# jinggqu/NextGen-UIA

Measured on AMD Instinct MI355X. Metric: images/sec fwd+bwd BiomedCLIP+Mona bs=256, higher is better.
Workload: dtype bf16

## Files before the change

### nextgen-uia_amd/csrc/wgrad.hip

```cpp
#include "uia_common.h"
#include "uia_kernels.h"

namespace {

typedef __attribute__((ext_vector_type(4))) short s16x4;
typedef __attribute__((ext_vector_type(8))) short s16x8;

__device__ __forceinline__ void glds16(const char* gsrc, char* lds_wave_base) {
    __builtin_amdgcn_global_load_lds((const __attribute__((address_space(1))) void*)gsrc,
                                     (__attribute__((address_space(3))) void*)lds_wave_base, 16, 0, 0);
}
__device__ __forceinline__ s16x4 lds_tr16(const char* p) {
    return __builtin_amdgcn_ds_read_tr16_b64_v4i16((__attribute__((address_space(3))) s16x4*)p);
}

constexpr int SLAB = 128;
#ifndef WG_CHUNK_SLABS
#define WG_CHUNK_SLABS 4
#endif
constexpr int CHUNK_SLABS = WG_CHUNK_SLABS;

#ifndef WG_MIN_WAVES
#define WG_MIN_WAVES 1
#endif
struct WgradGroups {
    const bf16_t* A[4];
    const bf16_t* B[4];
    float* dW[4];
    float* dbias[4];
    unsigned long long seed[4];
};

template <bool DROPB>
__global__ __launch_bounds__(256, DROPB ? 3 : WG_MIN_WAVES) void wgrad_bf16_kernel(int M, int I, int J, const WgradGroups gp, long lda, long ldb, float alpha,
                                                          long ldw, int i_valid, int j_valid, float drop_p, long drop_ld, int drop_col0) {
    extern __shared__ __attribute__((aligned(16))) char smem[];
    const bf16_t* __restrict__ A = gp.A[blockIdx.y];
    const bf16_t* __restrict__ B = gp.B[blockIdx.y];
    float* __restrict__ dW = gp.dW[blockIdx.y];
    float* __restrict__ dbias = gp.dbias[blockIdx.y];
    const unsigned long long drop_seed = gp.seed[blockIdx.y];
    char* As = smem;
    char* Bs = smem + SLAB * 128;
    const int tid = threadIdx.x, lane = tid & 63;
    const int wave = __builtin_amdgcn_readfirstlane(tid >> 6);
    const int tiles = (I / 64) * (J / 64);
    const int xcd = blockIdx.x & 7, slot = blockIdx.x >> 3;
    const int chunk = xcd + 8 * (slot / tiles), tile = slot % tiles;
    const int tj = tile % (J / 64), ti = tile / (J / 64);
    const int m_begin = chunk * (SLAB * CHUNK_SLABS);
    if (m_begin >= M) return;
    const int li = lane & 15, g = lane >> 4, qq = li >> 2, pp = li & 3;

    f32x4 acc[4][4];
#pragma unroll
    for (int a = 0; a < 4; ++a)
#pragma unroll
        for (int b = 0; b < 4; ++b) acc[a][b] = f32x4{0.f, 0.f, 0.f, 0.f};
    const bool want_bias = dbias != nullptr && tj == 0;
    f32x4 bacc[4] = {f32x4{0.f, 0.f, 0.f, 0.f}, f32x4{0.f, 0.f, 0.f, 0.f}, f32x4{0.f, 0.f, 0.f, 0.f}, f32x4{0.f, 0.f, 0.f, 0.f}};
    const bf16x8 ones = {(bf16_t)1.f, (bf16_t)1.f, (bf16_t)1.f, (bf16_t)1.f, (bf16_t)1.f, (bf16_t)1.f, (bf16_t)1.f, (bf16_t)1.f};

    const uint32_t drop_th = dropout_thresh16(drop_p);
    const float drop_inv = 1.0f / (1.0f - drop_p);
    const int trow = 32 * wave + 4 * g + qq;
    const int tsw = (trow >> 1) & 3;
    for (int sl = 0; sl < CHUNK_SLABS; ++sl) {
        const int m0 = m_begin + sl * SLAB;
        if (m0 >= M) break;
        __syncthreads();
        if constexpr (DROPB) {
            uint4 raw[SLAB / 32];
            uint32_t keep[SLAB / 32];
#pragma unroll
            for (int i = 0; i < SLAB / 32; ++i) {
                const int q = wave + 4 * i, r = 8 * q + (lane >> 3);
                int gm = m0 + r;
                gm = gm < M ? gm : M - 1;
                const int c = ((lane & 7) ^ (((r >> 1) & 3) << 1)) * 16;
                glds16((const char*)(A + (size_t)gm * lda + (size_t)ti * 64) + c, As + q * 1024);
                raw[i] = *(const uint4*)((const char*)(B + (size_t)gm * ldb + (size_t)tj * 64) + c);
            }
#pragma unroll
            for (int i = 0; i < SLAB / 32; ++i) {
                const int q = wave + 4 * i, r = 8 * q + (lane >> 3);
                int gm = m0 + r;
                gm = gm < M ? gm : M - 1;
                const int c = ((lane & 7) ^ (((r >> 1) & 3) << 1)) * 16;
                keep[i] = dropout_keep8(drop_seed, (uint32_t)(((size_t)gm * (size_t)drop_ld + (size_t)(drop_col0 + tj * 64 + (c >> 1))) >> 3), drop_th);
            }
#pragma unroll
            for (int i = 0; i < SLAB / 32; ++i) {
                const int q = wave + 4 * i;
                bf16x8 v = __builtin_bit_cast(bf16x8, raw[i]);
#pragma unroll
                for (int e = 0; e < 8; ++e) v[e] = (bf16_t)((keep[i] >> e) & 1u ? (float)v[e] * drop_inv : 0.f);
                *(bf16x8*)(Bs + q * 1024 + lane * 16) = v;
            }
        } else {
        for (int q = wave; q < SLAB / 8; q += 4) {
            const int r = 8 * q + (lane >> 3);
            int gm = m0 + r;
            gm = gm < M ? gm : M - 1;
            const int c = ((lane & 7) ^ (((r >> 1) & 3) << 1)) * 16;
            glds16((const char*)(A + (size_t)gm * lda + (size_t)ti * 64) + c, As + q * 1024);
            glds16((const char*)(B + (size_t)gm * ldb + (size_t)tj * 64) + c, Bs + q * 1024);
        }
        }
        asm volatile("s_waitcnt vmcnt(0)" ::: "memory");
        __syncthreads();
        const bool tail = m0 + SLAB > M;
        bf16x8 af[4], bfr[4];
#pragma unroll
        for (int t = 0; t < 4; ++t) {
            const int off = trow * 128 + ((t ^ tsw) << 5) + 8 * pp;
            s16x4 alo = lds_tr16(As + off), ahi = lds_tr16(As + off + 16 * 128);
            const s16x4 blo = lds_tr16(Bs + off), bhi = lds_tr16(Bs + off + 16 * 128);
            if (tail) {
#pragma unroll
                for (int e = 0; e < 4; ++e) {
                    if (m0 + 32 * wave + 4 * g + e >= M) alo[e] = 0;
                    if (m0 + 32 * wave + 16 + 4 * g + e >= M) ahi[e] = 0;
                }
            }
            const s16x8 av = {alo[0], alo[1], alo[2], alo[3], ahi[0], ahi[1], ahi[2], ahi[3]};
            const s16x8 bv = {blo[0], blo[1], blo[2], blo[3], bhi[0], bhi[1], bhi[2], bhi[3]};
            af[t] = __builtin_bit_cast(bf16x8, av);
            bfr[t] = __builtin_bit_cast(bf16x8, bv);
        }
#pragma unroll
        for (int a = 0; a < 4; ++a)
#pragma unroll
            for (int b = 0; b < 4; ++b) acc[a][b] = __builtin_amdgcn_mfma_f32_16x16x32_bf16(af[a], bfr[b], acc[a][b], 0, 0, 0);
        if (want_bias) {
#pragma unroll
            for (int a = 0; a < 4; ++a) bacc[a] = __builtin_amdgcn_mfma_f32_16x16x32_bf16(af[a], ones, bacc[a], 0, 0, 0);
        }
    }
    __syncthreads();
    float* red = (float*)smem;
    float* mine = red + (wave & 1) * 4096;
    if (wave < 2) {
#pragma unroll
        for (int a = 0; a < 4; ++a)
#pragma unroll
            for (int b = 0; b < 4; ++b)
#pragma unroll
                for (int r = 0; r < 4; ++r)
                    mine[(16 * a + 4 * g + r) * 64 + 16 * b + li] = acc[a][b][r];
    }
    __syncthreads();
    if (wave >= 2) {
#pragma unroll
        for (int a = 0; a < 4; ++a)
#pragma unroll
            for (int b = 0; b < 4; ++b)
#pragma unroll
                for (int r = 0; r < 4; ++r)
                    mine[(16 * a + 4 * g + r) * 64 + 16 * b + li] += acc[a][b][r];
    }
    __syncthreads();
#ifndef WG_NO_ATOMIC
    for (int e = tid; e < 4096; e += 256) {
        const float v = red[e] + red[4096 + e];
        const int i = ti * 64 + (e >> 6), j = tj * 64 + (e & 63);
        if (i < i_valid && j < j_valid) atomicAdd(dW + (size_t)i * ldw + j, v * alpha);
    }
#endif
    if (want_bias) {
        __syncthreads();
        if (li == 0) {
#pragma unroll
            for (int a = 0; a < 4; ++a)
#pragma unroll
                for (int r = 0; r < 4; ++r) red[wave * 64 + 16 * a + 4 * g + r] = bacc[a][r];
        }
        __syncthreads();
        if (tid < 64 && ti * 64 + tid < i_valid) atomicAdd(dbias + ti * 64 + tid, (red[tid] + red[64 + tid]) + (red[128 + tid] + red[192 + tid]));
    }
}

__global__ __launch_bounds__(256) void wgrad_f32_kernel(int M, int I, int J, const float* __restrict__ A, long lda,
                                                         const float* __restrict__ B, long ldb, float alpha,
                                                         float* __restrict__ dW, float* __restrict__ dbias, long ldw, int i_valid, int j_valid) {
    extern __shared__ __attribute__((aligned(16))) char smem[];
    const int tid = threadIdx.x, lane = tid & 63;
    const int wave = __builtin_amdgcn_readfirstlane(tid >> 6);
    const int tj = blockIdx.x % (J / 64), ti = blockIdx.x / (J / 64);
    const int m_begin = blockIdx.y * (SLAB * CHUNK_SLABS);
    const int m_end = min(M, m_begin + SLAB * CHUNK_SLABS);
    const int li = lane & 15, g = lane >> 4;
    f32x4 acc[4][4];
#pragma unroll
    for (int a = 0; a < 4; ++a)
#pragma unroll
        for (int b = 0; b < 4; ++b) acc[a][b] = f32x4{0.f, 0.f, 0.f, 0.f};
    float bsum = 0.f;
    for (int m = m_begin + 4 * wave; m < m_end; m += 16) {
        const int row = m + g;
        const bool ok = row < m_end;
        const int rr = ok ? row : m_end - 1;
        float av[4], bv[4];
#pragma unroll
        for (int t = 0; t < 4; ++t) {
            av[t] = ok ? A[(size_t)rr * lda + ti * 64 + 16 * t + li] : 0.f;
            bv[t] = B[(size_t)rr * ldb + tj * 64 + 16 * t + li];
            bsum += av[t];
        }
#pragma unroll
        for (int a = 0; a < 4; ++a)
#pragma unroll
            for (int b = 0; b < 4; ++b) acc[a][b] = __builtin_amdgcn_mfma_f32_16x16x4f32(av[a], bv[b], acc[a][b], 0, 0, 0);
        (void)bsum;
    }
    __syncthreads();
    float* red = (float*)smem;
#pragma unroll
    for (int a = 0; a < 4; ++a)
#pragma unroll
        for (int b = 0; b < 4; ++b)
#pragma unroll
            for (int r = 0; r < 4; ++r) red[wave * 4096 + (16 * a + 4 * g + r) * 64 + 16 * b + li] = acc[a][b][r];
    __syncthreads();
    for (int e = tid; e < 4096; e += 256) {
        const float v = red[e] + red[4096 + e] + red[8192 + e] + red[12288 + e];
        const int i = ti * 64 + (e >> 6), j = tj * 64 + (e & 63);
        if (i < i_valid && j < j_valid) atomicAdd(dW + (size_t)i * ldw + j, v * alpha);
    }
    if (dbias && tj == 0) {
        const int col = tid & 63, part = tid >> 6;
        float s = 0.f;
        for (int m = m_begin + part; m < m_end; m += 4) s += A[(size_t)m * lda + ti * 64 + col];
        __syncthreads();
        red[tid] = s;
        __syncthreads();
        if (tid < 64 && ti * 64 + tid < i_valid) atomicAdd(dbias + ti * 64 + tid, red[tid] + red[64 + tid] + red[128 + tid] + red[192 + tid]);
    }
}

}

int uia_wgrad_group_launch(hipStream_t stream, int dtype, int n, int M, int I, int J, const void* const* A, long lda, const void* const* B, long ldb, float alpha,
                            float* const* dW, float* const* dbias, long ldw, int i_valid, int j_valid, float drop_p, const uint64_t* drop_seed, long drop_ld, int drop_col0) {
    if (ldw == 0) { ldw = J; i_valid = I; j_valid = J; }
    UIA_CHECK_ARG(dtype == UIA_BF16 || dtype == UIA_F32, "uia_wgrad: bad dtype %d", dtype);
    UIA_CHECK_ARG(n >= 1 && n <= 4 && (n == 1 || dtype == UIA_BF16), "uia_wgrad_group: 1..4 problems per launch (bf16), got %d", n);
    UIA_CHECK_ARG(M > 0 && I > 0 && J > 0 && I % 64 == 0 && J % 64 == 0, "uia_wgrad: I=%d and J=%d must be multiples of 64 (M=%d)", I, J, M);
    const int esz = dtype == UIA_BF16 ? 2 : 4;
    UIA_CHECK_ARG((lda * esz) % 16 == 0 && (ldb * esz) % 16 == 0, "uia_wgrad: alignment");
    UIA_CHECK_ARG(lda >= I && ldb >= J, "uia_wgrad: leading dimension too small");
    UIA_CHECK_ARG(i_valid > 0 && i_valid <= I && j_valid > 0 && j_valid <= J && ldw >= j_valid, "uia_wgrad: valid extent %d x %d (ldw %ld) outside the padded %d x %d", i_valid, j_valid, ldw, I, J);
    WgradGroups gp = {};
    for (int g = 0; g < n; ++g) {
        UIA_CHECK_ARG(A[g] && B[g] && dW[g] && (uintptr_t)A[g] % 16 == 0 && (uintptr_t)B[g] % 16 == 0, "uia_wgrad: null or misaligned tensor (problem %d)", g);
        gp.A[g] = (const bf16_t*)A[g]; gp.B[g] = (const bf16_t*)B[g]; gp.dW[g] = dW[g]; gp.dbias[g] = dbias ? dbias[g] : nullptr; gp.seed[g] = drop_seed ? drop_seed[g] : 0;
    }
    const int chunks = (M + SLAB * CHUNK_SLABS - 1) / (SLAB * CHUNK_SLABS);
    const dim3 grid_f32((I / 64) * (J / 64), chunks);
    const dim3 grid(8 * ((chunks + 7) / 8) * (I / 64) * (J / 64), n);
    const int lds = 4 * 4096 * 4;
    const int lds_bf16 = 2 * SLAB * 128;
    static UiaDevOnce once_bf16, once_f32;
    UIA_CHECK_ARG(drop_p >= 0.f && drop_p < 1.f, "uia_wgrad: drop_p=%f outside [0, 1)", (double)drop_p);
    UIA_CHECK_ARG(drop_p == 0.f || (dtype == UIA_BF16 && drop_ld >= drop_col0 + J && drop_col0 >= 0 && drop_col0 % 8 == 0 && drop_ld % 8 == 0 && (size_t)M * (size_t)drop_ld / 8 <= 0xFFFFFFFFull),
                  "uia_wgrad: dropout on the B operand needs bf16, a window of J columns at a multiple of 8 inside rows of drop_ld (a multiple of 8) elements, M*drop_ld <= 2^35");
    UIA_ENSURE_LDS_ATTR(once_bf16, wgrad_bf16_kernel<false>, lds_bf16);
    UIA_ENSURE_LDS_ATTR(once_f32, wgrad_f32_kernel, lds);
    if (dtype == UIA_BF16)
        if (drop_p > 0.f) {
            static UiaDevOnce once_drop;
            UIA_ENSURE_LDS_ATTR(once_drop, wgrad_bf16_kernel<true>, lds_bf16);
            hipLaunchKernelGGL(wgrad_bf16_kernel<true>, grid, dim3(256), lds_bf16, stream, M, I, J, gp, lda, ldb, alpha, ldw, i_valid, j_valid, drop_p, drop_ld, drop_col0);
        } else
        hipLaunchKernelGGL(wgrad_bf16_kernel<false>, grid, dim3(256), lds_bf16, stream, M, I, J, gp, lda, ldb, alpha, ldw, i_valid, j_valid, 0.f, 0l, 0);
    else
        hipLaunchKernelGGL(wgrad_f32_kernel, grid_f32, dim3(256), lds, stream, M, I, J, (const float*)A[0], lda, (const float*)B[0], ldb, alpha, dW[0], dbias ? dbias[0] : nullptr, ldw, i_valid, j_valid);
    UIA_CHECK_LAUNCH();
    return 0;
}

int uia_wgrad_launch(hipStream_t stream, int dtype, int M, int I, int J, const void* A, long lda, const void* B, long ldb, float alpha,
                     float* dW, float* dbias, long ldw, int i_valid, int j_valid, float drop_p, uint64_t drop_seed, long drop_ld, int drop_col0) {
    UIA_CHECK_ARG(A && B && dW, "uia_wgrad: null tensor");
    return uia_wgrad_group_launch(stream, dtype, 1, M, I, J, &A, lda, &B, ldb, alpha, &dW, &dbias, ldw, i_valid, j_valid, drop_p, &drop_seed, drop_ld, drop_col0);
}
```

### nextgen-uia_amd/uia_hip/ops.py

```python
import ctypes as C
from typing import NamedTuple

import torch

from . import _lib
from ._lib import AttnDesc, GemmDesc, LnLoraDesc, LoraRankDesc, MonaFusedDesc, MonaSpatialDesc, PackDesc, UiaError, WgradGroupDesc, check, lib

_ACT = {None: 0, "none": 0, "gelu": 1, "quick_gelu": 2, "relu": 3}

GEMM_PROFILE = None


EPI_BIAS, EPI_AUX_OUT, EPI_GELU, EPI_DGELU, EPI_RESID, EPI_RESIDT, EPI_OUT32, EPI_OUTT, EPI_RESID_LN, EPI_GENERIC = 1, 2, 4, 8, 16, 32, 64, 128, 256, -1
EPI_QUICK = 2048
EPI_ROWSUM, EPI_LNFOLD = 512, 1024
EPI_RESID_LO, EPI_OUT_LO = 4096, 8192
_SPECIALISED = {EPI_BIAS | EPI_RESID | EPI_OUT32, EPI_BIAS | EPI_RESIDT | EPI_OUT32, EPI_BIAS | EPI_RESID | EPI_RESID_LN | EPI_OUT32, EPI_OUTT, EPI_BIAS | EPI_OUTT, EPI_BIAS | EPI_GELU | EPI_OUTT, EPI_DGELU | EPI_OUTT,
                EPI_BIAS | EPI_GELU | EPI_AUX_OUT | EPI_OUTT,
                EPI_QUICK | EPI_BIAS | EPI_GELU | EPI_OUTT, EPI_QUICK | EPI_DGELU | EPI_OUTT, EPI_QUICK | EPI_BIAS | EPI_GELU | EPI_AUX_OUT | EPI_OUTT,
                EPI_BIAS | EPI_RESID | EPI_OUT32 | EPI_OUTT | EPI_ROWSUM, EPI_BIAS | EPI_RESID | EPI_RESID_LN | EPI_OUT32 | EPI_OUTT | EPI_ROWSUM,
                EPI_BIAS | EPI_OUTT | EPI_LNFOLD, EPI_BIAS | EPI_GELU | EPI_OUTT | EPI_LNFOLD, EPI_BIAS | EPI_GELU | EPI_AUX_OUT | EPI_OUTT | EPI_LNFOLD,
                EPI_QUICK | EPI_BIAS | EPI_GELU | EPI_OUTT | EPI_LNFOLD, EPI_QUICK | EPI_BIAS | EPI_GELU | EPI_AUX_OUT | EPI_OUTT | EPI_LNFOLD,
                EPI_BIAS | EPI_RESID_LO | EPI_RESID_LN | EPI_OUTT | EPI_OUT_LO | EPI_ROWSUM,
                EPI_BIAS | EPI_RESID | EPI_OUTT | EPI_OUT_LO | EPI_ROWSUM, EPI_BIAS | EPI_RESID_LO | EPI_OUT32,
# ... 545 lines not shown
        d.splitk_ws = _p(splitk_ws)
    ext = w if isinstance(w, ExtW) else None
    if ext is not None:
        t2, gcols = a2
        d.A2, d.lda2, d.K2 = t2.data_ptr(), t2.stride(-2), ext.K2
        d.a2_group_cols, d.a2_group_stride = (gcols, t2.stride(0)) if t2.dim() == 3 else (0, 0)
    if drop is not None:
        d.drop_where, d.drop_p, d.drop_seed = {"a": 1, "acc": 2}[drop[0]], float(drop[1]), int(drop[2]) & 0xFFFFFFFFFFFFFFFF
        if len(drop) > 3 and drop[3] is not None:
            xo = drop[3]
            if drop[0] != "a" or xo.dtype != a.dtype or xo.shape != a.shape or xo.stride() != a.stride():
                raise UiaError("gemm drop: a_drop_out must have a's dtype, shape and strides")
            d.a_drop_out = _p(xo)
    packed = w if isinstance(w, PackedW) else None
    if ext is not None:
        d.lda, d.ldw, d.M, d.K, d.N = _rowmajor(a, "a"), ext.K, a.shape[0], ext.K, ext.N
        d.A = _p(a)
    else:
        wrow = packed.row if packed is not None else w
        d.ldw = _rowmajor(wrow, "w")
        if is_kb(a):
            d.M, d.K, d.a_kb_rows = _kb_dims(a, "gemm a")
            d.lda = d.K
        else:
            d.lda = _rowmajor(a, "a")
            d.M, d.K = a.shape[0], a.shape[1]
        if a.dtype != wrow.dtype or d.K != wrow.shape[1]:
            raise UiaError(f"gemm operand mismatch: a {(d.M, d.K)} {a.dtype}, w {tuple(wrow.shape)} {wrow.dtype}")
        d.A = _p(a.t if is_kb(a) else a)
        d.N = wrow.shape[0]
    esz = a.element_size()
    if launch is None:
        launch = plan_gemm(d.M, d.N, d.K, esz, 0, tile_cfg, whole=True,
                           **_plan_facts(a, w, act, dact, aux_out, out_group, resid_mod, drop, alpha, out_t, out32, resid, resid_t, rowsum, lnfold, resid_ln))[0]
    tile_cfg, base_cfg = launch.tile_cfg, launch.base
    d.W, d.w_kblocked = (_p(ext.kb if ext is not None else packed.kblocked()), 1) if launch.w_kblocked else (_p(wrow), 0)
    d.alpha = alpha
    d.act, d.dact = _ACT[act], _ACT[dact]
    if bias is not None:
        assert bias.dtype == torch.float32 and bias.numel() == d.N
        d.bias = _p(bias)
    for name, t, want in (("aux_in", aux_in, a.dtype), ("aux_out", aux_out, a.dtype), ("resid_t", resid_t, a.dtype),
                          ("resid", resid, torch.float32), ("out32", out32, torch.float32)):
        if t is not None and t.dtype != want:
            raise UiaError(f"gemm {name} must be {want}, got {t.dtype}")
    for name, t in (("aux_in", aux_in), ("aux_out", aux_out), ("resid_t", resid_t), ("out32", out32)):
        if t is not None and (t.dim() != 2 or t.shape[1] < d.N or (t.shape[0] < d.M and out_group == 0)):
            raise UiaError(f"gemm {name} is {tuple(t.shape)}: too small for the [{d.M}, {d.N}] result")
    if resid is not None and resid_mod == 0 and out_group == 0 and (resid.dim() != 2 or resid.shape[1] < d.N or resid.shape[0] < d.M):
        raise UiaError(f"gemm resid is {tuple(resid.shape)}: too small for the [{d.M}, {d.N}] result")
    if aux_in is not None:
        d.aux_in, d.ldaux_in = _p(aux_in), _rowmajor(aux_in, "aux_in")
    if aux_out is not None:
        d.aux_out, d.ldaux_out = _p(aux_out), _rowmajor(aux_out, "aux_out")
    if resid is not None:
        d.resid, d.ldr = _p(resid), _rowmajor(resid, "resid")
    d.resid_mod, d.resid_row_off, d.out_group = resid_mod, resid_row_off, out_group
    if resid_ln is not None:
        st, lw, lb = resid_ln[:3]
        if len(resid_ln) > 3:
            d.resid_ln_dim, d.resid_ln_eps = int(resid_ln[3]), float(resid_ln[4])
        if (resid is None and resid3 is None) or resid_mod or out_group:
            raise UiaError("gemm resid_ln needs a plain fp32 resid or a three-byte resid3 (no row remapping)")
        want_st = torch.int64 if len(resid_ln) > 3 else torch.float32
        if not (st.dtype == want_st and lw.dtype == lb.dtype == torch.float32 and st.is_contiguous() and st.numel() >= 2 * d.M and lw.numel() >= d.N and lb.numel() >= d.N):
            raise UiaError(f"gemm resid_ln: stats {tuple(st.shape)} / weight {tuple(lw.shape)} / bias {tuple(lb.shape)} do not cover [{d.M}, {d.N}]")
        d.resid_ln_stats, d.resid_ln_w, d.resid_ln_b = _p(st), _p(lw), _p(lb)
    if rowsum is not None:
        if not (rowsum.dtype == torch.int64 and rowsum.is_contiguous() and rowsum.numel() >= 2 * d.M) or out_group:
            raise UiaError(f"gemm rowsum must be a contiguous int64 [{d.M}, 2] tensor (no row remapping), got {tuple(rowsum.shape)} {rowsum.dtype}")
        d.rowsum_out = _p(rowsum)
    if lnfold is not None:
        sm, cs, dim, eps = lnfold
        if not (sm.dtype == torch.int64 and cs.dtype == torch.float32 and sm.is_contiguous() and cs.is_contiguous() and sm.numel() >= 2 * d.M and cs.numel() >= d.N) or alpha != 1.0:
            raise UiaError(f"gemm lnfold: sums {tuple(sm.shape)} {sm.dtype} / colsum {tuple(cs.shape)} do not cover [{d.M}, {d.N}] (int64 row sums, fp32 colsum, contiguous, alpha == 1)")
        d.lnfold_sums, d.lnfold_colsum, d.lnfold_dim, d.lnfold_eps = _p(sm), _p(cs), int(dim), float(eps)
    if (rowsum is not None or lnfold is not None) and a.is_cuda:
        d.ln_flag, d.ln_flag_limit = _p(ln_flag(a.device)), LN_FLAG_LIMIT
    if resid_t is not None:
        d.residT, d.ldrT = _p(resid_t), _rowmajor(resid_t, "resid_t")
    if resid3 is not None:
        if resid is not None or resid_t is not None:
            raise UiaError("gemm: resid3 replaces resid / resid_t")
        t, d.ldrT, d.residT_kb_rows = _plane(resid3[0], "resid3 hi plane", d.M, d.N, torch.bfloat16)
        d.residT = _p(t)
        t, d.ld_resid_lo, d.resid_lo_kb_rows = _plane(resid3[1], "resid3 low bytes", d.M, d.N, torch.int8)
        d.resid_lo8 = _p(t)
    if out_lo is not None:
        if out_t is None:
            raise UiaError("gemm out_lo needs out_t (the hi plane)")
        t, d.ld_out_lo, d.out_lo_kb_rows = _plane(out_lo, "out_lo", d.M, d.N, torch.int8)
        d.out_lo8 = _p(t)
    if out_t is not None:
        if out_group and is_kb(out_t):
            raise UiaError(f"gemm out_t (K-blocked {tuple(out_t.t.shape)}) does not hold the [{d.M}, {d.N}] result of a row-remapping launch")
        t, d.ldo, d.outT_kb_rows = _plane(out_t, "out_t", d.M, d.N, a.dtype, not out_group)
        d.outT = _p(t)
    if out32 is not None:
        d.out32, d.ldo32 = _p(out32), _rowmajor(out32, "out32")
    if GEMM_PROFILE is not None:
        e0, e1 = torch.cuda.Event(enable_timing=True), torch.cuda.Event(enable_timing=True)
        e0.record()
        check(lib().uia_gemm(_stream(), _code(a.dtype), C.byref(d), tile_cfg), "uia_gemm")
        e1.record()
        nbytes = esz * (d.M * d.K + d.N * d.K) + d.M * d.N * (esz * sum(t is not None for t in (aux_in, aux_out, resid_t, out_t))
                                                             + 4 * sum(t is not None for t in (resid, out32)) + 3 * (resid3 is not None) + 1 * (out_lo is not None))
        mask = epi_mask_of(d)
        if not (tile_cfg & 255) and base_cfg != 23:
            base_cfg = auto_tile_cfg(d.M, d.N, d.K, esz, mask)
        GEMM_PROFILE.append((e0, e1, d.M, d.N, d.K, a.dtype, base_cfg, nbytes, mask))
        return
    if _TRACE_GENERIC is not None:
        mask = epi_mask_of(d)
        if mask not in _SPECIALISED and d.M > 2048:
            _TRACE_GENERIC[(mask, d.M, d.N, d.K, base_cfg)] = _TRACE_GENERIC.get((mask, d.M, d.N, d.K, base_cfg), 0) + 1
    check(lib().uia_gemm(_stream(), _code(a.dtype), C.byref(d), tile_cfg), "uia_gemm")


def three_byte_to_float(hi, lo):
    h = hi.t.permute(1, 0, 2).reshape(hi.rows, hi.cols) if is_kb(hi) else hi
    lo = lo.t.permute(1, 0, 2).reshape(lo.rows, lo.cols) if is_kb(lo) else lo
    h = h[:lo.shape[0], :lo.shape[1]]
    bits = (h.contiguous().view(torch.int16).to(torch.int32) << 16) + (lo.to(torch.int32) << 8)
    return bits.view(torch.float32)


def float_to_three_byte(x):
    hi = x.bfloat16()
    xb = x.contiguous().view(torch.int32).to(torch.int64) & 0xFFFFFFFF
    hb = hi.contiguous().view(torch.int16).to(torch.int64) & 0xFFFF
    d = ((xb + 0x80) >> 8) - (hb << 8)
    return hi, d.clamp(-127, 127).to(torch.int8)


def wgrad(a, b, dw, dbias=None, alpha=1.0, drop=None):
    lda, ldb = _rowmajor(a, "a"), _rowmajor(b, "b")
    assert a.dtype == b.dtype and a.shape[0] == b.shape[0] and dw.dtype == torch.float32 and dw.is_contiguous() and dw.dim() == 2
    I, J = a.shape[1], b.shape[1]
    if drop is not None:
        p, seed = drop
        if dbias is not None or a.dtype != torch.bfloat16 or ldb != J:
            raise UiaError("wgrad(drop=...): bf16, no bias, and b must be the whole dropped tensor (contiguous rows)")
        check(lib().uia_wgrad_drop(_stream(), _code(a.dtype), a.shape[0], I, J, _p(a), lda, _p(b), ldb, alpha, _p(dw), dw.shape[1], dw.shape[0], dw.shape[1],
                                   float(p), int(seed) & 0xFFFFFFFFFFFFFFFF, J, 0), "uia_wgrad_drop")
        return
    if tuple(dw.shape) == (I, J):
        check(lib().uia_wgrad(_stream(), _code(a.dtype), a.shape[0], I, J, _p(a), lda, _p(b), ldb, alpha, _p(dw), _p(dbias)), "uia_wgrad")
        return
    assert dw.shape[0] <= I and dw.shape[1] <= J and (dbias is None or dbias.numel() >= dw.shape[0])
    check(lib().uia_wgrad_ex(_stream(), _code(a.dtype), a.shape[0], I, J, _p(a), lda, _p(b), ldb, alpha, _p(dw), dw.shape[1], dw.shape[0], dw.shape[1],
                             _p(dbias)), "uia_wgrad_ex")


LORA_WGRAD_GROUP = True


def wgrad_group(a_list, b_list, dw_list, dbias_list=None, alpha=1.0, drop=None):
    n = len(a_list)
    a0, b0, w0 = a_list[0], b_list[0], dw_list[0]
    if not (1 <= n <= 4 and len(b_list) == n and len(dw_list) == n and a0.dtype == torch.bfloat16):
        raise UiaError("wgrad_group: 1..4 bf16 problems")
    lda, ldb = _rowmajor(a0, "a"), _rowmajor(b0, "b")
    M, I, J = a0.shape[0], a0.shape[1], b0.shape[1]
    d = WgradGroupDesc()
    d.n, d.M, d.I, d.J, d.lda, d.ldb, d.ldw = n, M, I, J, lda, ldb, w0.shape[1]
    d.i_valid, d.j_valid, d.alpha = w0.shape[0], w0.shape[1], alpha
    for g in range(n):
        a, b, w = a_list[g], b_list[g], dw_list[g]
        if (a.dtype != torch.bfloat16 or b.dtype != torch.bfloat16 or tuple(a.shape) != (M, I) or tuple(b.shape) != (M, J) or _rowmajor(a, "a") != lda or _rowmajor(b, "b") != ldb
                or w.dtype != torch.float32 or not w.is_contiguous() or w.shape != w0.shape or w.shape[0] > I or w.shape[1] > J):
            raise UiaError(f"wgrad_group: problem {g} does not have the shape / strides / dtypes of problem 0")
        d.A[g], d.B[g], d.dW[g] = a.data_ptr(), b.data_ptr(), w.data_ptr()
        db = dbias_list[g] if dbias_list is not None else None
        if db is not None:
            assert db.dtype == torch.float32 and db.numel() >= w.shape[0]
            d.dbias_A[g] = db.data_ptr()
    if drop is not None:
        p_, seeds = drop
        if ldb != J or (dbias_list is not None and any(x is not None for x in dbias_list)):
            raise UiaError("wgrad_group(drop=...): no bias, and each b must be the whole dropped tensor (contiguous rows)")
        d.drop_p, d.drop_ld, d.drop_col0 = float(p_), J, 0
        for g in range(n):
            d.drop_seed[g] = int(seeds[g]) & 0xFFFFFFFFFFFFFFFF
    check(lib().uia_wgrad_group(_stream(), _code(a0.dtype), C.byref(d)), "uia_wgrad_group")


def _attn_desc(q, k, v, out, lse, B, H, L, mask, keylen, scale, dh=None):
    d = AttnDesc()
    for t in (q, k, v):
        if t.stride(-1) != 1 or t.dtype != q.dtype:
            raise UiaError("attention operands must be unit-stride in the last dim and share a dtype")
    width = q.shape[-1]
    if width % H != 0 or (dh is not None and dh * H != width) or k.shape[-1] != width or v.shape[-1] != width:
        raise UiaError(f"attention: q / k / v are {q.shape[-1]} / {k.shape[-1]} / {v.shape[-1]} columns wide for {H} heads" + (f" of dim {dh}" if dh is not None else ""))
    dh = width // H
    if dh not in (16, 32, 64):
        raise UiaError(f"attention: head dim {dh} unsupported (16, 32 or 64): {width} columns over {H} heads")
    if not is_kb(out) and out.shape[-1] != width:
        raise UiaError(f"attention: out is {out.shape[-1]} columns wide, q / k / v {width}")
    d.q, d.k, d.v, d.ld_qkv = _p(q), _p(k), _p(v), q.stride(-2)
    assert k.stride(-2) == q.stride(-2) == v.stride(-2)
    if is_kb(out):
        rows, cols, d.out_kb_rows = _kb_dims(out, "attention out")
        if rows < B * L or cols != H * dh or dh != 64 or q.dtype != torch.bfloat16:
            raise UiaError(f"attention out (K-blocked {tuple(out.t.shape)}) must hold [{B * L}, {H * dh}] bf16 with head dim 64")
        d.out, d.ldo = _p(out.t), cols
    else:
        d.out, d.ldo = _p(out), out.stride(-2)
    d.lse = _p(lse)
    d.keylen = _p(keylen)
    d.B, d.H, d.L, d.dh = B, H, L, dh
    d.mask_kind = {"none": 0, None: 0, "causal": 1, "keypad": 2}[mask]
    d.scale = scale if scale is not None else dh ** -0.5
    return d


def attn_fwd(q, k, v, out, B, H, L, lse=None, mask=None, keylen=None, scale=None, dh=None, cu_seqlens=None):
    d = _attn_desc(q, k, v, out, lse, B, H, L, mask, keylen, scale, dh)
    if cu_seqlens is not None:
        assert cu_seqlens.dtype == torch.int32 and cu_seqlens.is_contiguous() and cu_seqlens.numel() == B + 1
        d.cu_seqlens = _p(cu_seqlens)
    check(lib().uia_attn_fwd(_stream(), _code(q.dtype), C.byref(d)), "uia_attn_fwd")


def attn_fwd_long(q, k, v, out, B, H, L, lse=None, scale=None):
    if is_kb(out):
        raise UiaError("attn_fwd_long: the output must be a row-major tensor, not K-blocked")
    d = _attn_desc(q, k, v, out, lse, B, H, L, None, None, scale)
    if d.dh != 64:
        raise UiaError(f"attn_fwd_long: head dim {d.dh}, only 64 is supported")
    check(lib().uia_attn_fwd_long(_stream(), _code(q.dtype), C.byref(d)), "uia_attn_fwd_long")


ATTN_BWD_CFG = 0


def attn_bwd(q, k, v, out, dout, lse, dq, dk, dv, B, H, L, mask=None, keylen=None, scale=None, dh=None, cfg=None):
    d = _attn_desc(q, k, v, out, lse, B, H, L, mask, keylen, scale, dh)
    dh = d.dh
    d.dout, d.lddo = _p(dout), dout.stride(-2)
    if is_kb(dq):
        rows, cols, d.dqkv_kb_rows = _kb_dims(dq, "attention dqkv")
        if rows < B * L or cols != 3 * H * dh or dh != 64 or q.dtype != torch.bfloat16 or dk is not None or dv is not None:
            raise UiaError(f"attention dqkv (K-blocked {tuple(dq.t.shape)}) must hold [{B * L}, {3 * H * dh}] bf16 with head dim 64, dk = dv = None")
        part = (H * dh // kb_group(q.dtype)) * d.dqkv_kb_rows * kb_group(q.dtype) * dq.t.element_size()
        d.dq, d.dk, d.dv, d.ld_dqkv = dq.t.data_ptr(), dq.t.data_ptr() + part, dq.t.data_ptr() + 2 * part, cols
    else:
        d.dq, d.dk, d.dv, d.ld_dqkv = _p(dq), _p(dk), _p(dv), dq.stride(-2)
        assert dk.stride(-2) == dq.stride(-2) == dv.stride(-2)
    cfg = ATTN_BWD_CFG if cfg is None else cfg
    if cfg:
        check(lib().uia_attn_bwd_cfg(_stream(), _code(q.dtype), C.byref(d), int(cfg)), "uia_attn_bwd_cfg")
    else:
        check(lib().uia_attn_bwd(_stream(), _code(q.dtype), C.byref(d)), "uia_attn_bwd")


def attn_bwd_cls(q, k, v, out, dout, lse, dq, dk, dv, B, H, L, mask=None, scale=None, rows=False):
    if mask not in (None, "none"):
        raise UiaError(f"attn_bwd_cls: mask {mask!r}: the CLS-query backward takes unmasked attention only")
    d = _attn_desc(q, k, v, out, lse, B, H, L, None, None, scale)
    if d.dh != 64:
        raise UiaError(f"attn_bwd_cls: head dim {d.dh}, only 64 is supported")
    if dout.dim() != 2 or dout.shape[0] != B or dout.shape[1] != H * 64 or dout.stride(1) != 1 or dout.dtype != q.dtype:
        raise UiaError(f"attn_bwd_cls: dout must be [{B}, {H * 64}] {q.dtype} rows (one per sequence), got {tuple(dout.shape)} {dout.dtype}")
    compact = bool(rows)
    if compact and (is_kb(out) or out.dim() != 2 or out.shape[0] != B or out.stride(1) != 1 or out.dtype != q.dtype):
        raise UiaError(f"attn_bwd_cls(rows=True): out must be [{B}, {H * 64}] {q.dtype} rows (one per sequence)")
    if lse is None or lse.dtype != torch.float32 or not lse.is_contiguous() or lse.numel() != (B * H if compact else B * H * L):
        raise UiaError(f"attn_bwd_cls: lse must be a contiguous fp32 [{B}, {H}, {L}] tensor ([{B}, {H}] beside a compact out)")
    d.dout, d.lddo = _p(dout), dout.stride(0)
    if is_kb(dq):
        rows, cols, d.dqkv_kb_rows = _kb_dims(dq, "attention dqkv")
        if rows < B * L or cols != 3 * H * 64 or q.dtype != torch.bfloat16 or dk is not None or dv is not None:
            raise UiaError(f"attention dqkv (K-blocked {tuple(dq.t.shape)}) must hold [{B * L}, {3 * H * 64}] bf16 with head dim 64, dk = dv = None")
        part = (H * 64 // kb_group(q.dtype)) * d.dqkv_kb_rows * kb_group(q.dtype) * dq.t.element_size()
        d.dq, d.dk, d.dv, d.ld_dqkv = dq.t.data_ptr(), dq.t.data_ptr() + part, dq.t.data_ptr() + 2 * part, cols
    else:
        for name, t in (("dq", dq), ("dk", dk), ("dv", dv)):
            if t.dtype != q.dtype or t.dim() != 2 or t.shape[0] < B * L or t.shape[1] != H * 64 or t.stride(1) != 1 or t.stride(0) != dq.stride(0):
                raise UiaError(f"attn_bwd_cls: {name} must be [{B * L}, {H * 64}] {q.dtype} rows sharing one row stride, got {tuple(t.shape)} {t.dtype}")
        d.dq, d.dk, d.dv, d.ld_dqkv = _p(dq), _p(dk), _p(dv), dq.stride(0)
    if compact:
        check(lib().uia_attn_bwd_cls_rows(_stream(), _code(q.dtype), C.byref(d)), "uia_attn_bwd_cls_rows")
    else:
        check(lib().uia_attn_bwd_cls(_stream(), _code(q.dtype), C.byref(d)), "uia_attn_bwd_cls")


def attn_fwd_cls(q, k, v, out, B, H, L, lse=None, mask=None, keylen=None, scale=None):
    if mask not in (None, "none", "keypad"):
        raise UiaError(f"attn_fwd_cls: mask {mask!r}: none or key padding only")
    if is_kb(out) or out.dim() != 2 or out.shape[0] != B or out.shape[1] != H * 64 or out.stride(1) != 1 or out.dtype != q.dtype:
        raise UiaError(f"attn_fwd_cls: out must be [{B}, {H * 64}] {q.dtype} rows (one per sequence)")
    if q.shape[0] < B * L:
        raise UiaError(f"attn_fwd_cls: q / k / v hold {q.shape[0]} rows, {B} sequences of {L} need {B * L}")
    if lse is not None and (lse.dtype != torch.float32 or not lse.is_contiguous() or lse.numel() != B * H):
        raise UiaError(f"attn_fwd_cls: lse must be a contiguous fp32 [{B}, {H}] tensor")
    if mask == "keypad" and (keylen is None or keylen.dtype != torch.int32 or not keylen.is_contiguous() or keylen.numel() != B):
        raise UiaError(f"attn_fwd_cls: key padding needs keylen int32 [{B}]")
    d = _attn_desc(q, k, v, out, lse, B, H, L, mask, keylen if mask == "keypad" else None, scale)
    if d.dh != 64:
        raise UiaError(f"attn_fwd_cls: head dim {d.dh}, only 64 is supported")
    check(lib().uia_attn_fwd_cls(_stream(), _code(q.dtype), C.byref(d)), "uia_attn_fwd_cls")


def rows3_to_f32(hi, lo, stride_rows, dst):
    rows, D = dst.shape
# ... 1434 lines not shown
```

Before: 6851.

## Add multi-buffered row-split wgrad kernel with async LDS pipeline for non-dropout bf16

Replaces the non-dropout bf16 weight-gradient kernel with a new kernel that keeps a four-deep ring of 64-row LDS slabs, issuing global-to-LDS loads several slabs ahead and waiting on partial vmcnt so loads overlap the MFMA work. Each wave now owns a 16-row strip of the 64x64 tile instead of the whole tile, and the rows-per-workgroup plan sizes M chunks from the tile count so small-tile problems get more parallel chunks. This removes the serial load-then-compute stall of the old single-buffer loop and shrinks the cross-wave reduction, at the cost of more LDS, more atomics per output when there are more chunks, and inline asm that touches m0. The dropout path is split into its own kernel and left unchanged.

```diff
diff --git a/nextgen-uia_amd/csrc/wgrad.hip b/nextgen-uia_amd/csrc/wgrad.hip
--- a/nextgen-uia_amd/csrc/wgrad.hip
+++ b/nextgen-uia_amd/csrc/wgrad.hip
@@ -15,14 +15,8 @@
 }
 
 constexpr int SLAB = 128;
-#ifndef WG_CHUNK_SLABS
-#define WG_CHUNK_SLABS 4
-#endif
-constexpr int CHUNK_SLABS = WG_CHUNK_SLABS;
-
-#ifndef WG_MIN_WAVES
-#define WG_MIN_WAVES 1
-#endif
+constexpr int CHUNK_SLABS = 4;
+
 struct WgradGroups {
     const bf16_t* A[4];
     const bf16_t* B[4];
@@ -31,9 +25,8 @@
     unsigned long long seed[4];
 };
 
-template <bool DROPB>
-__global__ __launch_bounds__(256, DROPB ? 3 : WG_MIN_WAVES) void wgrad_bf16_kernel(int M, int I, int J, const WgradGroups gp, long lda, long ldb, float alpha,
-                                                          long ldw, int i_valid, int j_valid, float drop_p, long drop_ld, int drop_col0) {
+__global__ __launch_bounds__(256, 3) void wgrad_drop_kernel(int M, int I, int J, const WgradGroups gp, long lda, long ldb, float alpha,
+                                                            long ldw, int i_valid, int j_valid, float drop_p, long drop_ld, int drop_col0) {
     extern __shared__ __attribute__((aligned(16))) char smem[];
     const bf16_t* __restrict__ A = gp.A[blockIdx.y];
     const bf16_t* __restrict__ B = gp.B[blockIdx.y];
@@ -69,7 +62,7 @@
         const int m0 = m_begin + sl * SLAB;
         if (m0 >= M) break;
         __syncthreads();
-        if constexpr (DROPB) {
+        {
             uint4 raw[SLAB / 32];
             uint32_t keep[SLAB / 32];
 #pragma unroll
@@ -97,15 +90,6 @@
                 for (int e = 0; e < 8; ++e) v[e] = (bf16_t)((keep[i] >> e) & 1u ? (float)v[e] * drop_inv : 0.f);
                 *(bf16x8*)(Bs + q * 1024 + lane * 16) = v;
             }
-        } else {
-        for (int q = wave; q < SLAB / 8; q += 4) {
-            const int r = 8 * q + (lane >> 3);
-            int gm = m0 + r;
-            gm = gm < M ? gm : M - 1;
-            const int c = ((lane & 7) ^ (((r >> 1) & 3) << 1)) * 16;
-            glds16((const char*)(A + (size_t)gm * lda + (size_t)ti * 64) + c, As + q * 1024);
-            glds16((const char*)(B + (size_t)gm * ldb + (size_t)tj * 64) + c, Bs + q * 1024);
-        }
         }
         asm volatile("s_waitcnt vmcnt(0)" ::: "memory");
         __syncthreads();
@@ -160,13 +144,11 @@
                     mine[(16 * a + 4 * g + r) * 64 + 16 * b + li] += acc[a][b][r];
     }
     __syncthreads();
-#ifndef WG_NO_ATOMIC
     for (int e = tid; e < 4096; e += 256) {
         const float v = red[e] + red[4096 + e];
         const int i = ti * 64 + (e >> 6), j = tj * 64 + (e & 63);
         if (i < i_valid && j < j_valid) atomicAdd(dW + (size_t)i * ldw + j, v * alpha);
     }
-#endif
     if (want_bias) {
         __syncthreads();
         if (li == 0) {
@@ -177,6 +159,124 @@
         }
         __syncthreads();
         if (tid < 64 && ti * 64 + tid < i_valid) atomicAdd(dbias + ti * 64 + tid, (red[tid] + red[64 + tid]) + (red[128 + tid] + red[192 + tid]));
+    }
+}
+
+__device__ __forceinline__ void glds16_ring(const char* gsrc, char* lds_wave_base) {
+    const unsigned dst_u = __builtin_amdgcn_readfirstlane((unsigned)(uintptr_t)(__attribute__((address_space(3))) char*)lds_wave_base);
+    unsigned keep;
+    asm volatile("s_mov_b32 %0, m0\n\ts_mov_b32 m0, %2\n\ts_nop 0\n\tglobal_load_lds_dwordx4 %1, off\n\ts_mov_b32 m0, %0"
+                 : "=&s"(keep) : "v"(gsrc), "s"(dst_u) : "memory");
+}
+
+constexpr int RS_SLAB = 64;
+constexpr int RS_NBUF = 4;
+constexpr int RS_OPER = RS_SLAB * 128;
+constexpr int RS_SLAB_BYTES = 2 * RS_OPER;
+constexpr int RS_PIECES = 2 * (RS_SLAB / 8) / 4;
+constexpr int RS_LDS = RS_NBUF * RS_SLAB_BYTES;
+
+__global__ __launch_bounds__(256, 2) void wgrad_rows_kernel(int M, int I, int J, const WgradGroups gp, long lda, long ldb, float alpha,
+                                                            long ldw, int i_valid, int j_valid, int rows_per_wg) {
+    extern __shared__ __attribute__((aligned(16))) char smem[];
+    const bf16_t* __restrict__ A = gp.A[blockIdx.y];
+    const bf16_t* __restrict__ B = gp.B[blockIdx.y];
+    float* __restrict__ dW = gp.dW[blockIdx.y];
+    float* __restrict__ dbias = gp.dbias[blockIdx.y];
+    const int tid = threadIdx.x, lane = tid & 63;
+    const int wave = __builtin_amdgcn_readfirstlane(tid >> 6);
+    const int tiles = (I / 64) * (J / 64);
+    const int xcd = blockIdx.x & 7, slot = blockIdx.x >> 3;
+    const int chunk = xcd + 8 * (slot / tiles), tile = slot % tiles;
+    const int tj = tile % (J / 64), ti = tile / (J / 64);
+    const long m_begin = (long)chunk * rows_per_wg;
+    if (m_begin >= M) return;
+    const int rows = (int)min((long)rows_per_wg, (long)M - m_begin);
+    const int nsl = (rows + RS_SLAB - 1) / RS_SLAB;
+    const int li = lane & 15, g = lane >> 4, qq = li >> 2, pp = li & 3;
+
+    const int prow = lane >> 3;
+    const int pcol = ((lane & 7) ^ (((prow >> 1) & 3) << 1)) * 16;
+    const char* Ab = (const char*)(A + (size_t)ti * 64) + pcol;
+    const char* Bb = (const char*)(B + (size_t)tj * 64) + pcol;
+    auto stage = [&](int t) {
+        char* buf = smem + (t % RS_NBUF) * RS_SLAB_BYTES;
+        const long m0 = m_begin + (long)t * RS_SLAB;
+#pragma unroll
+        for (int i = 0; i < RS_SLAB / 32; ++i) {
+            const int q = wave + 4 * i;
+            long gm = m0 + 8 * q + prow;
+            gm = gm < M ? gm : (long)M - 1;
+            glds16_ring(Ab + (size_t)gm * (size_t)lda * 2, buf + q * 1024);
+            glds16_ring(Bb + (size_t)gm * (size_t)ldb * 2, buf + RS_OPER + q * 1024);
+        }
+    };
+
+    f32x4 acc[4] = {f32x4{0.f, 0.f, 0.f, 0.f}, f32x4{0.f, 0.f, 0.f, 0.f}, f32x4{0.f, 0.f, 0.f, 0.f}, f32x4{0.f, 0.f, 0.f, 0.f}};
+    f32x4 bacc = f32x4{0.f, 0.f, 0.f, 0.f};
+    const bool want_bias = dbias != nullptr && tj == 0;
+    const bf16x8 ones = {(bf16_t)1.f, (bf16_t)1.f, (bf16_t)1.f, (bf16_t)1.f, (bf16_t)1.f, (bf16_t)1.f, (bf16_t)1.f, (bf16_t)1.f};
+    const int tsw = ((4 * g + qq) >> 1) & 3;
+    const int frow = (4 * g + qq) * 128 + 8 * pp;
+
+    constexpr int PD = RS_NBUF - 1;
+    for (int t = 0; t < PD && t < nsl; ++t) stage(t);
+    for (int s = 0; s < nsl; ++s) {
+        const int younger = min(nsl - 1 - s, PD - 1);
+        if (younger >= 2) asm volatile("s_waitcnt vmcnt(%0)" ::"n"(2 * RS_PIECES) : "memory");
+        else if (younger == 1) asm volatile("s_waitcnt vmcnt(%0)" ::"n"(RS_PIECES) : "memory");
+        else asm volatile("s_waitcnt vmcnt(0)" ::: "memory");
+        asm volatile("s_waitcnt lgkmcnt(0)" ::: "memory");
+        __builtin_amdgcn_s_barrier();
+        __builtin_amdgcn_sched_barrier(0);
+        if (s + PD < nsl) stage(s + PD);
+        const char* As = smem + (s % RS_NBUF) * RS_SLAB_BYTES;
+        const char* Bs = As + RS_OPER;
+        const int left = rows - s * RS_SLAB;
+#pragma unroll
+        for (int ks = 0; ks < RS_SLAB / 32; ++ks) {
+            const int base = ks * 32 * 128 + frow;
+            s16x4 alo = lds_tr16(As + base + ((wave ^ tsw) << 5)), ahi = lds_tr16(As + base + ((wave ^ tsw) << 5) + 16 * 128);
+            bf16x8 bfr[4];
+#pragma unroll
+            for (int b = 0; b < 4; ++b) {
+                const s16x4 blo = lds_tr16(Bs + base + ((b ^ tsw) << 5)), bhi = lds_tr16(Bs + base + ((b ^ tsw) << 5) + 16 * 128);
+                const s16x8 bv = {blo[0], blo[1], blo[2], blo[3], bhi[0], bhi[1], bhi[2], bhi[3]};
+                bfr[b] = __builtin_bit_cast(bf16x8, bv);
+            }
+            if (left < RS_SLAB) {
+#pragma unroll
+                for (int e = 0; e < 4; ++e) {
+                    if (32 * ks + 4 * g + e >= left) alo[e] = 0;
+                    if (32 * ks + 16 + 4 * g + e >= left) ahi[e] = 0;
+                }
+            }
+            const s16x8 av = {alo[0], alo[1], alo[2], alo[3], ahi[0], ahi[1], ahi[2], ahi[3]};
+            const bf16x8 af = __builtin_bit_cast(bf16x8, av);
+#pragma unroll
+            for (int b = 0; b < 4; ++b) acc[b] = __builtin_amdgcn_mfma_f32_16x16x32_bf16(af, bfr[b], acc[b], 0, 0, 0);
+            if (want_bias) bacc = __builtin_amdgcn_mfma_f32_16x16x32_bf16(af, ones, bacc, 0, 0, 0);
+        }
+    }
+    asm volatile("s_waitcnt vmcnt(0) lgkmcnt(0)" ::: "memory");
+    __syncthreads();
+    float* red = (float*)smem;
+#pragma unroll
+    for (int b = 0; b < 4; ++b)
+#pragma unroll
+        for (int r = 0; r < 4; ++r)
+            red[(16 * wave + 4 * g + r) * 64 + 16 * b + li] = acc[b][r];
+    __syncthreads();
+    for (int e = tid; e < 4096; e += 256) {
+        const int i = ti * 64 + (e >> 6), j = tj * 64 + (e & 63);
+        if (i < i_valid && j < j_valid) atomicAdd(dW + (size_t)i * ldw + j, red[e] * alpha);
+    }
+    if (want_bias && li == 0) {
+#pragma unroll
+        for (int r = 0; r < 4; ++r) {
+            const int i = ti * 64 + 16 * wave + 4 * g + r;
+            if (i < i_valid) atomicAdd(dbias + i, bacc[r]);
+        }
     }
 }
 
@@ -236,6 +336,14 @@
         __syncthreads();
         if (tid < 64 && ti * 64 + tid < i_valid) atomicAdd(dbias + ti * 64 + tid, red[tid] + red[64 + tid] + red[128 + tid] + red[192 + tid]);
     }
+}
+
+int wgrad_rows_plan(int M, int I, int J, int n) {
+    const int tiles = (I / 64) * (J / 64) * n;
+    const int per_xcd = tiles >= 64 ? 1 : (64 / tiles > 6 ? 6 : 64 / tiles);
+    const int chunks = 8 * per_xcd;
+    const int rows = ((M + chunks - 1) / chunks + RS_SLAB - 1) / RS_SLAB * RS_SLAB;
+    return rows > 512 ? rows : 512;
 }
 
 }
@@ -257,23 +365,26 @@
     }
     const int chunks = (M + SLAB * CHUNK_SLABS - 1) / (SLAB * CHUNK_SLABS);
     const dim3 grid_f32((I / 64) * (J / 64), chunks);
-    const dim3 grid(8 * ((chunks + 7) / 8) * (I / 64) * (J / 64), n);
     const int lds = 4 * 4096 * 4;
-    const int lds_bf16 = 2 * SLAB * 128;
-    static UiaDevOnce once_bf16, once_f32;
+    static UiaDevOnce once_bf16, once_drop, once_f32;
     UIA_CHECK_ARG(drop_p >= 0.f && drop_p < 1.f, "uia_wgrad: drop_p=%f outside [0, 1)", (double)drop_p);
     UIA_CHECK_ARG(drop_p == 0.f || (dtype == UIA_BF16 && drop_ld >= drop_col0 + J && drop_col0 >= 0 && drop_col0 % 8 == 0 && drop_ld % 8 == 0 && (size_t)M * (size_t)drop_ld / 8 <= 0xFFFFFFFFull),
                   "uia_wgrad: dropout on the B operand needs bf16, a window of J columns at a multiple of 8 inside rows of drop_ld (a multiple of 8) elements, M*drop_ld <= 2^35");
-    UIA_ENSURE_LDS_ATTR(once_bf16, wgrad_bf16_kernel<false>, lds_bf16);
     UIA_ENSURE_LDS_ATTR(once_f32, wgrad_f32_kernel, lds);
-    if (dtype == UIA_BF16)
+    if (dtype == UIA_BF16) {
         if (drop_p > 0.f) {
-            static UiaDevOnce once_drop;
-            UIA_ENSURE_LDS_ATTR(once_drop, wgrad_bf16_kernel<true>, lds_bf16);
-            hipLaunchKernelGGL(wgrad_bf16_kernel<true>, grid, dim3(256), lds_bf16, stream, M, I, J, gp, lda, ldb, alpha, ldw, i_valid, j_valid, drop_p, drop_ld, drop_col0);
-        } else
-        hipLaunchKernelGGL(wgrad_bf16_kernel<false>, grid, dim3(256), lds_bf16, stream, M, I, J, gp, lda, ldb, alpha, ldw, i_valid, j_valid, 0.f, 0l, 0);
-    else
+            const int lds_drop = 2 * SLAB * 128;
+            const dim3 grid(8 * ((chunks + 7) / 8) * (I / 64) * (J / 64), n);
+            UIA_ENSURE_LDS_ATTR(once_drop, wgrad_drop_kernel, lds_drop);
+            hipLaunchKernelGGL(wgrad_drop_kernel, grid, dim3(256), lds_drop, stream, M, I, J, gp, lda, ldb, alpha, ldw, i_valid, j_valid, drop_p, drop_ld, drop_col0);
+        } else {
+            const int rows_per_wg = wgrad_rows_plan(M, I, J, n);
+            const int row_chunks = (M + rows_per_wg - 1) / rows_per_wg;
+            const dim3 grid(8 * ((row_chunks + 7) / 8) * (I / 64) * (J / 64), n);
+            UIA_ENSURE_LDS_ATTR(once_bf16, wgrad_rows_kernel, RS_LDS);
+            hipLaunchKernelGGL(wgrad_rows_kernel, grid, dim3(256), RS_LDS, stream, M, I, J, gp, lda, ldb, alpha, ldw, i_valid, j_valid, rows_per_wg);
+        }
+    } else
         hipLaunchKernelGGL(wgrad_f32_kernel, grid_f32, dim3(256), lds, stream, M, I, J, (const float*)A[0], lda, (const float*)B[0], ldb, alpha, dW[0], dbias ? dbias[0] : nullptr, ldw, i_valid, j_valid);
     UIA_CHECK_LAUNCH();
     return 0;
diff --git a/nextgen-uia_amd/uia_hip/ops.py b/nextgen-uia_amd/uia_hip/ops.py
--- a/nextgen-uia_amd/uia_hip/ops.py
+++ b/nextgen-uia_amd/uia_hip/ops.py
@@ -721,6 +721,12 @@
                              _p(dbias)), "uia_wgrad_ex")
 
 
+def wgrad_rows_per_workgroup(M, I, J, n=1):
+    tiles = (I // 64) * (J // 64) * n
+    chunks = 8 * (1 if tiles >= 64 else min(6, 64 // tiles))
+    return max(512, -(-(-(-M // chunks)) // 64) * 64)
+
+
 LORA_WGRAD_GROUP = True
 
 
```

After: 6861, median of 2. No clear change (+0.1%).
